# zenghjian/SceneSplat

Hardware: AMD Instinct MI355X
Metric: Gaussians/s encoder fwd+bwd, 102k-pt chunks (higher is better)
Workload: dtype bf16

## Files before the change

include/scenesplat_hip.h:

```cpp
#ifndef SCENESPLAT_HIP_H
#define SCENESPLAT_HIP_H
#include <stddef.h>
#include <stdint.h>

#ifdef __cplusplus
extern "C" {
#endif

struct ihipStream_t;
typedef struct ihipStream_t* ss_stream_t;

#define SS_MAX_ORDERS 8
enum { SS_ORDER_Z = 0, SS_ORDER_Z_TRANS = 1, SS_ORDER_HILBERT = 2, SS_ORDER_HILBERT_TRANS = 3 };
enum { SS_DTYPE_F32 = 0, SS_DTYPE_BF16 = 1 };
enum { SS_ATTN_SIMT = 0, SS_ATTN_MFMA = 1 };
enum { SS_OK = 0, SS_ERR_ARG = 1, SS_ERR_LAUNCH = 2, SS_ERR_WORKSPACE = 3 };

int ss_version(void);

int ss_serialize_encode(const int32_t* grid_coord, const int32_t* batch, int64_t n, int depth, const int* orders,
                        int num_orders, int64_t* codes, ss_stream_t stream);
int ss_offsets_to_batch(const int32_t* offsets, int num_batches, int64_t n, int32_t* batch, ss_stream_t stream);
int ss_count_duplicates(const int64_t* sorted_keys, int64_t n, int32_t* count, ss_stream_t stream);
int ss_grid_coord_max(const int32_t* grid_coord, int64_t n, int32_t* out_max, ss_stream_t stream);
// ... 61 lines not shown
int ss_window_attn_hm_bwd(const void* hm, const void* out, const void* dout, const float* neg_lse2, const int32_t* gidx,
                          const int32_t* sidx, const int32_t* win_start, int num_windows, int max_window, int64_t n,
                          int64_t n_pad, int channels, int num_heads, float scale, void* dqkv, void* workspace,
                          size_t workspace_bytes, ss_stream_t stream);

int ss_window_attn_rpe_fwd(const void* qkv, const int32_t* gidx, const int32_t* sidx, const int32_t* win_start,
                           int num_windows, int max_window, int64_t n, int64_t n_pad, int channels, int num_heads,
                           float scale, int dtype, int impl, const int32_t* grid_coord, const float* table, int pos_bnd,
                           void* out, float* lse, ss_stream_t stream);
size_t ss_window_attn_rpe_bwd_workspace_bytes(int64_t n, int64_t n_pad, int channels, int num_heads, int dtype,
                                              int num_windows, int max_window, int pos_bnd);
int ss_window_attn_rpe_bwd(const void* qkv, const void* out, const void* dout, const float* lse, const int32_t* gidx,
                           const int32_t* sidx, const int32_t* win_start, int num_windows, int max_window, int64_t n,
                           int64_t n_pad, int channels, int num_heads, float scale, int dtype, int impl,
                           const int32_t* grid_coord, const float* table, int pos_bnd, void* dqkv, float* dtable,
                           void* workspace, size_t workspace_bytes, ss_stream_t stream);

int ss_subm_rulebook(const int32_t* grid_coord, const int32_t* batch, int64_t n, int depth,
                     const int64_t* zkeys_sorted, const int32_t* zorder, int swap_xy, int kernel_size, int32_t* nbr,
                     ss_stream_t stream);
int ss_subm_tap_mask_keys(const int32_t* nbr, const int32_t* order, int64_t n, int taps, int coarse_bits, int64_t* keys,
                          ss_stream_t stream);
int64_t ss_subm_rulebook_table_size(int64_t n);
int ss_subm_rulebook_hashed(const int32_t* grid_coord, const int32_t* batch, int64_t n, int depth, int kernel_size, int32_t* nbr,
                            void* workspace, size_t workspace_bytes, ss_stream_t stream);

int ss_subm_conv_fwd(const void* in, const void* weight, const float* bias, const int32_t* nbr, const int32_t* rowperm,
                     void* out, int64_t n, int cin, int cout, int taps, int out_dtype, ss_stream_t stream);
int ss_subm_weight_mirror(const void* w, void* wt, int cout, int taps, int cin, ss_stream_t stream);
int ss_stream_create_cu_mask(int nwords, const uint32_t* mask, void** stream_out);
int ss_subm_im2col(const void* src, const int32_t* nbr, void* dst, int64_t n, int taps, int64_t row_bytes, ss_stream_t stream);
int ss_gemm8_ok(int64_t m, int k, int n, int taps);
int ss_subm_conv_fwd_pipe(const void* in, const void* weight, const float* bias, const int32_t* nbr, const int32_t* rowperm,
                          void* out, int64_t n, int cin, int cout, int taps, int out_dtype, ss_stream_t stream);
int ss_subm_conv_fwd_pipe_walk(const void* in, const void* weight, const float* bias, const int32_t* nbr_walk, const int32_t* rowperm,
                               void* out, int64_t n, int cin, int cout, int taps, int out_dtype, ss_stream_t stream);
int ss_subm_conv_fwd_uses_pipe(int64_t n, int cin, int cout, int taps);
int ss_subm_conv_fwd_walk(const void* in, const void* weight, const float* bias, const int32_t* nbr, const int32_t* nbr_walk,
                          const int32_t* rowperm, void* out, int64_t n, int cin, int cout, int taps, int out_dtype, ss_stream_t stream);
int ss_linear_fwd(const void* x, const void* weight, const float* bias, void* out, int64_t m, int k, int n, int out_dtype,
                  ss_stream_t stream);
int ss_wgrad_xcd_order(void);
int ss_wgrad_set_xcd_order(int on);
int ss_wgrad8_ok(int64_t n, int cin, int cout, int taps);
int ss_subm_conv_wgrad_pipe(const void* in, const void* dout, const int32_t* nbr, const int32_t* rowperm,
                            const int32_t* blk_count, const int32_t* blk_list, float* dweight, int64_t n, int cin, int cout,
                            int taps, ss_stream_t stream);
int ss_linear_wgrad(const void* x, const void* dy, float* dweight, float* dbias, int64_t m, int k_in, int n_out,
                    ss_stream_t stream);
int ss_linear_wgrad_group_plan(int64_t m, int k_in, int n_out, int64_t* desc_words);
int ss_linear_wgrad_tiles(int k_in, int n_out);
int ss_linear_wgrad_group_plan2(int64_t m, int k_in, int n_out, int launch_tiles, int64_t* desc_words);
int ss_linear_wgrad_group(const int64_t* desc, const int32_t* wg_start, int nprob, int total_workgroups, ss_stream_t stream);
int ss_subm_conv_splits(int64_t n, int cout, int taps);
int ss_subm_conv_fwd_splitk(const void* in, const void* weight, const float* bias, const int32_t* nbr, const int32_t* rowperm,
                            float* acc32, int64_t n, int cin, int cout, int taps, int splits, ss_stream_t stream);
int ss_subm_block_lists(const int32_t* nbr, const int32_t* rowperm, int64_t n, int taps, int32_t* blk_count,
                        int32_t* blk_list, ss_stream_t stream);
int ss_subm_conv_wgrad(const void* in, const void* dout, const int32_t* nbr, const int32_t* rowperm,
                       const int32_t* blk_count, const int32_t* blk_list, float* dweight, int64_t n, int cin, int cout,
                       int taps, ss_stream_t stream);

int ss_subm_f32_ok(int cin_padded, int cout);
int ss_subm_f32_fwd(const float* in, const float* wq, const float* bias, const int32_t* nbr_walk, const int32_t* rowperm,
                    float* out, int64_t n, int cin_padded, int cout, int taps, ss_stream_t stream);
int ss_subm_f32_dgrad_dup(const float* dout_folded, const float* wq, const int32_t* nbr_walk, const int32_t* rowperm, float* din,
                          int64_t n, int cin_padded, int cout, int taps, ss_stream_t stream);
int ss_subm_f32_wgrad(const float* in, const float* dout, const int32_t* nbr_walk, const int32_t* rowperm,
                      const int32_t* blk_count, const int32_t* blk_list, float* dweight, int64_t n, int cin_padded,
                      int cin, int cout, int taps, ss_stream_t stream);

int ss_subm_conv_wgrad_pipe_walk(const void* in, const void* dout, const int32_t* nbr_walk, const int32_t* rowperm,
                                 const int32_t* blk_count, const int32_t* blk_list, float* dweight, int64_t n, int cin, int cout,
                                 int taps, ss_stream_t stream);
int ss_subm_conv_wgrad_uses_pipe(int64_t n, int cin, int cout, int taps);
int ss_subm_conv_wgrad_walk(const void* in, const void* dout, const int32_t* nbr, const int32_t* nbr_walk, const int32_t* rowperm,
                            const int32_t* blk_count, const int32_t* blk_list, float* dweight, int64_t n, int cin, int cout,
                            int taps, ss_stream_t stream);

int ss_add_layernorm_fwd(const void* x, int x_dtype, const void* y, int y_dtype, const float* rowscale,
                         const float* gamma, const float* beta, float eps, void* xout, int xout_dtype, void* xcopy_bf16,
                         void* h, int h_dtype, float* mean, float* rstd, int64_t n, int channels, ss_stream_t stream);
int ss_ln_add_ln_fwd(const void* x, int x_dtype, const void* t, int t_dtype, const float* gamma0, const float* beta0, float eps0,
                     const float* gamma1, const float* beta1, float eps1, float* xout, void* h, int h_dtype, float* stats,
                     int64_t n, int channels, ss_stream_t stream);
int ss_ln_add_ln_bwd(const float* g_xout, const void* g_h, int g_h_dtype, const float* xout, const void* t, int t_dtype,
                     const float* stats, const float* gamma0, const float* gamma1, void* g_x, int g_x_dtype, void* g_t,
                     int g_t_dtype, float* part, int64_t n, int channels, int nblocks, ss_stream_t stream);
int ss_add_layernorm_bwd_blocks(int64_t n);

int ss_block_tail_rows(void);
int ss_block_tail_bwd_blocks(int64_t n);
int ss_block_tail_fwd(const void* feat, const float* x, const float* rs1, const float* rs2, const void* wp, const void* bp,
                      const void* w1, const void* b1, const void* w2, const void* b2, int bias_dtype, const float* gamma, const float* beta,
                      float eps, float* x_mid, float* mean, float* rstd, void* h2, void* u, void* a, float* x_out,
                      void* xcopy_bf16, int64_t n, int channels, ss_stream_t stream);
int ss_block_tail_bwd(const float* g_xout, const void* g_xcopy_bf16, const float* x_mid, const float* mean, const float* rstd,
                      const void* u, const float* rs1, const float* rs2, const float* gamma, const void* wp_t, const void* w1_t,
                      const void* w2_t, float* g_mid, void* dfeat, void* dy2, void* du, void* dy1, float* part, int64_t n,
                      int channels, int nblocks, ss_stream_t stream);
int ss_group_partial_sums_outputs_per_workgroup(void);
int ss_group_partial_sums(const int64_t* desc, const int32_t* wg_start, int nprob, int total_workgroups, ss_stream_t stream);
int ss_transpose16_group(const int64_t* desc, const int32_t* wg_start, int nprob, int total_workgroups, ss_stream_t stream);
int ss_subm_weight_mirror_group_tile(void);
int ss_subm_weight_mirror_group(const int64_t* desc, const int32_t* wg_start, int nprob, int total_workgroups, ss_stream_t stream);
int ss_add_layernorm_bwd(const void* g_xout, int g_xout_dtype, const void* g_xcopy, int g_xcopy_dtype, const void* g_h,
// ... 204 lines not shown
```

scenesplat_amd/csrc/wgrad8.hip:

```cpp
#include "grouped.h"
#include <stdlib.h>

typedef __attribute__((ext_vector_type(8))) __bf16 w8_bf8_t;
typedef __attribute__((ext_vector_type(4))) short w8_s4_t;
typedef __attribute__((ext_vector_type(8))) short w8_s8_t;
typedef __attribute__((address_space(3))) w8_s4_t w8_lds_s4_t;
#define W8_MFMA(a, b, c) __builtin_amdgcn_mfma_f32_16x16x32_bf16((a), (b), (c), 0, 0, 0)

#define W8_BUF 65536
#define W8_HALF 16384
#define W8_OFF_B 32768
#define W8_CHUNK 60
#define W8_OFF_ISITE 131072
#define W8_OFF_JSITE (W8_OFF_ISITE + W8_CHUNK * 64 * 4)
#define W8_LDS_BYTES (W8_OFF_JSITE + W8_CHUNK * 64 * 4)
#define W8_ZERO_ELEMS 4096

__device__ uint4 w8_zero[W8_ZERO_ELEMS / 8];

__device__ __forceinline__ void w8_glds16(const void* gsrc, unsigned lds_wave_base) {
  asm volatile("s_mov_b32 m0, %1\n\ts_nop 0\n\tglobal_load_lds_dwordx4 %0, off" ::"v"(gsrc), "s"(lds_wave_base) : "memory");
}
__device__ __forceinline__ w8_bf8_t w8_tr2(const char* p) {
  w8_s4_t lo = __builtin_amdgcn_ds_read_tr16_b64_v4i16((w8_lds_s4_t*)(p));
// ... 239 lines not shown
      }
  if (do_bias && lq == 0) {
#pragma unroll
    for (int ha = 0; ha < 2; ++ha)
#pragma unroll
      for (int r = 0; r < 4; ++r) {
        const int co = m0 + 128 * wr + 64 * ha + 16 * wc + 4 * g + r;
        if (co < Cout) atomicAdd(dbias + co, accb[ha][r]);
      }
  }
}

#undef W8_BIAS

#define W8_XG 3
__device__ __forceinline__ int w8_xcd_order(int L, int nb) {
  const int row = 8 * W8_XG, full = nb / row * row;
  if (L >= full) return L;
  const int xcd = L & 7, slot = L >> 3;
  return ((slot / W8_XG) * 8 + xcd) * W8_XG + slot % W8_XG;
}

template <bool GATHER>
__global__ void __launch_bounds__(512)
k_wgrad8(const unsigned short* __restrict__ X, const unsigned short* __restrict__ DY, const int32_t* __restrict__ nbr,
         const int32_t* __restrict__ rowperm, const int32_t* __restrict__ blk_count, const int32_t* __restrict__ blk_list,
         float* __restrict__ dW, float* __restrict__ dbias, int n, int Cin, int Cout, int taps, int ntn, int nblocks_total,
         int min_per, int ntiles, int nshares, int walk) {
  int L = (int)blockIdx.x;
  if (walk & 2) L = w8_xcd_order(L, (int)gridDim.x);
  w8_body<GATHER>(X, DY, nbr, rowperm, blk_count, blk_list, dW, dbias, n, Cin, Cout, taps, ntn, nblocks_total, min_per, ntiles,
                  nshares, L, walk & 1);
}

__global__ void __launch_bounds__(512)
k_wgrad8_group(const int64_t* __restrict__ desc, const int32_t* __restrict__ wg_start, int nprob, int nprob_flags) {
  const int b = blockIdx.x;
  const int p = group_owner(wg_start, nprob, b);
  const int64_t* d = desc + (int64_t)p * 8;
  const int64_t m = d[4];
  const uint64_t w5 = (uint64_t)d[5], w6 = (uint64_t)d[6], w7 = (uint64_t)d[7];
  const int k_in = (int)(w5 & 0xffffffffu), n_out = (int)(w5 >> 32);
  const int ntn = (int)(w6 & 0xffffffffu), ntiles = (int)(w6 >> 32);
  const int nshares = (int)(w7 & 0xffffffffu), min_per = (int)(w7 >> 32);
  int L = b - wg_start[p];
  if (nprob_flags & 1) {
    const int a = (8 - (wg_start[p] & 7)) & 7;
    if (L >= a) L = a + w8_xcd_order(L - a, nshares * ntiles - a);
  }
  w8_body<false>((const unsigned short*)d[0], (const unsigned short*)d[1], nullptr, nullptr, nullptr, nullptr, (float*)d[2],
                 (float*)d[3], (int)m, k_in, n_out, 1, ntn, (int)((m + 63) / 64), min_per, ntiles, nshares, L);
}

static int w8_xcd_flag = -1;
extern "C" int ss_wgrad_xcd_order(void) {
  if (w8_xcd_flag < 0) { const char* e = getenv("SS_WGRAD_XCD_TRIPLE"); w8_xcd_flag = (e && atoi(e) == 1) ? 1 : 0; }
  return w8_xcd_flag;
}
extern "C" int ss_wgrad_set_xcd_order(int on) { w8_xcd_flag = on ? 1 : 0; return SS_OK; }

extern "C" int ss_wgrad8_ok(int64_t n, int cin, int cout, int taps) {
  return n > 0 && n < (1LL << 31) && cin >= 8 && (cin & 7) == 0 && cin <= W8_ZERO_ELEMS && cout >= 8 && (cout & 7) == 0 &&
         cout <= W8_ZERO_ELEMS && taps >= 1;
}

static int w8_min_per(int64_t busy_tiles, int64_t est_blocks) {
  int64_t per = busy_tiles * est_blocks / 200;
  if (per < 8) per = 8;
  if (per > 160) per = 160;
  return (int)per;
}

static int w8_conv_launch(const void* in, const void* dout, const int32_t* nbr, const int32_t* rowperm, const int32_t* blk_count,
                          const int32_t* blk_list, float* dweight, int64_t n, int cin, int cout, int taps, int walk, hipStream_t stream);

extern "C" int ss_subm_conv_wgrad_pipe(const void* in, const void* dout, const int32_t* nbr, const int32_t* rowperm,
                                       const int32_t* blk_count, const int32_t* blk_list, float* dweight, int64_t n,
                                       int cin, int cout, int taps, hipStream_t stream) {
  return w8_conv_launch(in, dout, nbr, rowperm, blk_count, blk_list, dweight, n, cin, cout, taps, 0, stream);
}
extern "C" int ss_subm_conv_wgrad_pipe_walk(const void* in, const void* dout, const int32_t* nbr_walk, const int32_t* rowperm,
                                            const int32_t* blk_count, const int32_t* blk_list, float* dweight, int64_t n,
                                            int cin, int cout, int taps, hipStream_t stream) {
  return w8_conv_launch(in, dout, nbr_walk, rowperm, blk_count, blk_list, dweight, n, cin, cout, taps, 1, stream);
}

static int w8_conv_launch(const void* in, const void* dout, const int32_t* nbr, const int32_t* rowperm, const int32_t* blk_count,
                          const int32_t* blk_list, float* dweight, int64_t n, int cin, int cout, int taps, int walk, hipStream_t stream) {
  if (n == 0) return SS_OK;
  if (!ss_wgrad8_ok(n, cin, cout, taps) || !blk_count || !blk_list || !nbr) return SS_ERR_ARG;
  const int nblocks = ss_div_up(n, 64);
  const int tm = ss_div_up(cout, 256), tn = ss_div_up(cin, 256);
  static int env_per = -2;
  if (env_per == -2) { const char* e = getenv("SS_WGRAD_MINPER"); env_per = e ? atoi(e) : -1; }
  int min_per = env_per > 0 ? env_per : w8_min_per((int64_t)tm * tn * ((taps + 2) / 3), (int64_t)nblocks * 7 / 10);
  int splits = ss_div_up(nblocks, min_per);
  if (ss_wgrad_xcd_order()) walk |= 2;
  dim3 g((unsigned)((int64_t)taps * splits * tm * tn));
  SS_LAUNCH((k_wgrad8<true>), g, dim3(512), 0, stream, (const unsigned short*)in, (const unsigned short*)dout, nbr, rowperm,
            blk_count, blk_list, dweight, (float*)nullptr, (int)n, cin, cout, taps, tn, nblocks, min_per, tm * tn, splits, walk);
  return SS_OK;
}

static void w8_linear_plan(int64_t m, int k_in, int n_out, int* tm_, int* tn_, int* min_per_, int* splits_, int launch_tiles = 0) {
  const int nblocks = ss_div_up(m, 64);
  const int tm = ss_div_up(n_out, 256), tn = ss_div_up(k_in, 256);
  static int env_per = -2;
  if (env_per == -2) { const char* e = getenv("SS_WGRAD_MINPER"); env_per = e ? atoi(e) : -1; }
  static const int cus = [] {
    int dev = 0, n = 256;
    if (hipGetDevice(&dev) == hipSuccess) (void)hipDeviceGetAttribute(&n, hipDeviceAttributeMultiprocessorCount, dev);
    return n > 0 ? n : 256;
  }();
  const int tiles_all = launch_tiles > tm * tn ? launch_tiles : tm * tn;
  const int shares = cus / tiles_all > 0 ? cus / tiles_all : 1;
  int min_per = env_per > 0 ? env_per : (int)((nblocks + shares - 1) / shares);
  if (env_per <= 0 && min_per < 8) min_per = 8;
  if (min_per > nblocks) min_per = nblocks;
  *tm_ = tm; *tn_ = tn; *min_per_ = min_per; *splits_ = ss_div_up(nblocks, min_per);
}

extern "C" int ss_linear_wgrad_tiles(int k_in, int n_out) { return ss_div_up(n_out, 256) * ss_div_up(k_in, 256); }
extern "C" int ss_linear_wgrad_group_plan2(int64_t m, int k_in, int n_out, int launch_tiles, int64_t* desc_words) {
  if (m <= 0 || !ss_wgrad8_ok(m, k_in, n_out, 1) || !desc_words) return 0;
  int tm, tn, min_per, splits;
  w8_linear_plan(m, k_in, n_out, &tm, &tn, &min_per, &splits, launch_tiles);
  desc_words[5] = (int64_t)((uint64_t)(uint32_t)k_in | ((uint64_t)(uint32_t)n_out << 32));
  desc_words[6] = (int64_t)((uint64_t)(uint32_t)tn | ((uint64_t)(uint32_t)(tm * tn) << 32));
  desc_words[7] = (int64_t)((uint64_t)(uint32_t)splits | ((uint64_t)(uint32_t)min_per << 32));
  return splits * tm * tn;
}
extern "C" int ss_linear_wgrad_group_plan(int64_t m, int k_in, int n_out, int64_t* desc_words) {
  return ss_linear_wgrad_group_plan2(m, k_in, n_out, 0, desc_words);
}

extern "C" int ss_linear_wgrad_group(const int64_t* desc, const int32_t* wg_start, int nprob, int total_workgroups,
                                     hipStream_t stream) {
  SS_GROUP_GUARD(desc, wg_start, nprob, total_workgroups);
  if (nprob > 128) return SS_ERR_ARG;
  SS_LAUNCH(k_wgrad8_group, dim3((unsigned)total_workgroups), dim3(512), 0, stream, desc, wg_start, nprob, 0);
  return SS_OK;
}

extern "C" int ss_linear_wgrad(const void* x, const void* dy, float* dweight, float* dbias, int64_t m, int k_in, int n_out,
                               hipStream_t stream) {
  if (m == 0) return SS_OK;
  if (!ss_wgrad8_ok(m, k_in, n_out, 1)) return SS_ERR_ARG;
  const int nblocks = ss_div_up(m, 64);
  int tm, tn, min_per, splits;
  w8_linear_plan(m, k_in, n_out, &tm, &tn, &min_per, &splits);
  dim3 g((unsigned)(splits * tm * tn));
  SS_LAUNCH((k_wgrad8<false>), g, dim3(512), 0, stream, (const unsigned short*)x, (const unsigned short*)dy,
            (const int32_t*)nullptr, (const int32_t*)nullptr, (const int32_t*)nullptr, (const int32_t*)nullptr, dweight,
            dbias, (int)m, k_in, n_out, 1, tn, nblocks, min_per, tm * tn, splits, 0);
  return SS_OK;
}
```

scenesplat_amd/functional.py:

```python
import os
import weakref

import torch
from torch.utils.weak import WeakIdKeyDictionary

from . import native as nv


def _bf16_autocast(x=None):
    return (x is None or x.is_cuda) and torch.is_autocast_enabled() and torch.get_autocast_dtype("cuda") == torch.bfloat16


class _WindowAttention(torch.autograd.Function):
    @staticmethod
    def forward(ctx, qkv, win, num_heads, scale, impl):
        qkv = qkv.contiguous()
        out, lse = nv.window_attn_fwd(qkv, win, num_heads, scale, impl)
        ctx.save_for_backward(qkv, out, lse)
        ctx.win, ctx.num_heads, ctx.scale, ctx.impl = win, num_heads, scale, impl
        return out

    @staticmethod
    def backward(ctx, dout):
        qkv, out, lse = ctx.saved_tensors
# ... 495 lines not shown
        nv.subm_weight_mirror_group(pairs)


def register_mirrored(weights):
    for p in weights:
        ent = _SHADOW.get(p)
        if ent is not None and p.dim() == 5 and p.shape[-1] % 8 == 0:
            cout, cin = p.shape[0], p.shape[-1]
            ent.want("m", (cin, p.numel() // (cout * cin), cout), p.device)


def register_transposed(weights):
    for p in weights:
        ent = _SHADOW.get(p)
        if ent is not None and p.dim() == 2:
            ent.want("t", (p.shape[1], p.shape[0]), p.device)


def unregister_transposed(weights):
    for ent in filter(None, map(_SHADOW.get, weights)):
        ent.set("t", None)


def unregister_mirrored(weights):
    for ent in filter(None, map(_SHADOW.get, weights)):
        ent.set("m", None)


def mirrored_of(p):
    ent = _current(p)
    return ent.m if ent is not None else None


def bf16_t_of(p):
    ent = _current(p)
    return ent.t if ent is not None else None


def bf16_of(p):
    if p is None or p.dtype == torch.bfloat16:
        return p
    ent = _current(p)
    return ent.bf16 if ent is not None else p.to(torch.bfloat16)


WGRAD_GROUP_MAX_ROWS = int(os.environ.get("SS_WGRAD_GROUP_MAX", str(1 << 22)))
_STAGE = {"cur": None, "route": {}}
_UNFLUSHED = set()


WGRAD_GROUP_MAX_BYTES = int(float(os.environ.get("SS_WGRAD_GROUP_MAX_GIB", "8")) * (1 << 30))


class _WgradStage:
    def __init__(self):
        self.queue = []
        self.redq = []
        self.bytes = 0

    def add(self, x, dy, dw, db):
        self.queue.append((x, dy, dw, db))
        self.bytes += x.numel() * x.element_size() + dy.numel() * dy.element_size()
        if self.bytes > WGRAD_GROUP_MAX_BYTES:
            q, self.queue, self.bytes = self.queue, [], 0
            nv.linear_wgrad_group(q)

    def flush(self):
        _UNFLUSHED.discard(self)
        q, self.queue, self.bytes = self.queue, [], 0
        r, self.redq = self.redq, []
        nv.linear_wgrad_group(q)
        nv.group_partial_sums(r)


class _StageParams(torch.autograd.Function):
    @staticmethod
    def forward(ctx, stage, *params):
        ctx.stage = stage
        ctx.set_materialize_grads(False)
        return tuple(p.view_as(p) for p in params)

    @staticmethod
    def backward(ctx, *grads):
        ctx.stage.flush()
        return (None,) + grads


def stage_begin(linears, n_rows):
    _STAGE["cur"], _STAGE["route"] = None, {}
    if not (WGRAD_GROUP_MAX_ROWS and LINEAR_WGRAD_MIN_ROWS <= n_rows <= WGRAD_GROUP_MAX_ROWS and torch.is_grad_enabled() and _bf16_autocast()):
        return
    params = [p for m in linears for p in (m.weight, m.bias) if p is not None and p.requires_grad and p.dtype == torch.float32 and p.is_cuda]
    if not params:
        return
    stage = _WgradStage()
    aliases = _StageParams.apply(stage, *params)
    _STAGE["cur"], _STAGE["route"] = stage, {id(p): a for p, a in zip(params, aliases)}


def stage_end():
    _STAGE["cur"], _STAGE["route"] = None, {}


def reset_state():
    stage_end()
    _UNFLUSHED.clear()
    _HEAD_CACHE.clear()


def _routed(p):
    a = _STAGE["route"].get(id(p)) if (p is not None and _STAGE["route"]) else None
    return (a, _STAGE["cur"]) if a is not None else (p, None)


def _linear_operands(weight, bias, cast_bias=True):
    wr, stage = _routed(weight) if torch.is_grad_enabled() else (weight, None)
    br = _routed(bias)[0] if stage is not None else bias
    return wr, br, bf16_of(weight), bf16_of(bias) if cast_bias else None, stage, bf16_t_of(weight)


class _Linear(torch.autograd.Function):

    @staticmethod
    def forward(ctx, x, weight, bias, w16, b16, stage, w16t=None):
        y = torch.nn.functional.linear(x, w16, b16)
        _save_linear(ctx, x, weight, bias, w16, w16t, stage)
        return y

    @staticmethod
    def backward(ctx, dy):
        x, w16 = ctx.saved_tensors
        return _linear_backward_of(ctx, x, w16, dy.contiguous()) + (None,) * 4


class _LinearGelu(torch.autograd.Function):

    @staticmethod
    def forward(ctx, x, weight, bias, w16, b16, stage, w16t=None):
        u = torch.nn.functional.linear(x, w16, b16)
        _save_linear(ctx, x, weight, bias, w16, w16t, stage, u)
        return nv.gelu(u)

    @staticmethod
    def backward(ctx, dy):
        x, w16, u = ctx.saved_tensors
        dy = dy.contiguous()
        if not _aligned16(dy):
            dy = dy.clone()
        return _linear_backward_of(ctx, x, w16, nv.gelu(u, dy)) + (None,) * 4


def _save_linear(ctx, x, weight, bias, w16, w16t, stage, *more):
    ctx.save_for_backward(x, w16 if w16t is None else w16t, *more)
    ctx.meta, ctx.dgrad_nt, ctx.stage = (weight.dtype, bias is not None), w16t is not None, stage


def _linear_backward_of(ctx, x, w16, dy):
    w_dtype, has_bias = ctx.meta
    return _linear_backward(x, w16, ctx.dgrad_nt, w_dtype, has_bias, ctx.stage, dy, *ctx.needs_input_grad[:3])

# ... 475 lines not shown
```

scenesplat_amd/native.py:

```python
import ctypes

import numpy as np
import torch

from . import _lib, grouped
from ._lib import check

_C = _lib.CONSTANTS
F32, BF16 = _C["SS_DTYPE_F32"], _C["SS_DTYPE_BF16"]
ATTN_SIMT, ATTN_MFMA = _C["SS_ATTN_SIMT"], _C["SS_ATTN_MFMA"]
HAVE_MFMA_ATTN = True
ORDER_IDS = {name: _C["SS_ORDER_" + name.upper().replace("-", "_")] for name in ("z", "z-trans", "hilbert", "hilbert-trans")}


def _p(t):
    return ctypes.c_void_p(t.data_ptr()) if t is not None else ctypes.c_void_p(0)


def _stream():
    return ctypes.c_void_p(torch.cuda.current_stream().cuda_stream)


def _req(t, dtype=None, name="tensor", shape=None):
    if not isinstance(t, torch.Tensor) or not t.is_cuda:
# ... 305 lines not shown
def dup_fold_rows(src, runs):
    keys, order = runs
    n, C = src.shape
    _req(src, None, "src"); _req(keys, torch.int64, "sorted_keys", (n,)); _req(order, torch.int32, "order", (n,))
    out = torch.empty_like(src)
    check(lib().ss_dup_fold_rows(_p(src), _p(keys), _p(order), _p(out), n, C, dtype_code(src), _stream()), "ss_dup_fold_rows")
    return out


def dup_zero_rows_(x, runs):
    keys, order = runs
    n = x.shape[0]
    _req(x, None, "x"); _req(keys, torch.int64, "sorted_keys", (n,)); _req(order, torch.int32, "order", (n,))
    check(lib().ss_dup_zero_rows(_p(keys), _p(order), _p(x), n, x.shape[1] * x.element_size(), _stream()), "ss_dup_zero_rows")
    return x


def subm_f32_wgrad(x, dout, nbr, rowperm, blocks, cin):
    n, cp = x.shape
    taps = nbr.shape[0]
    _req(x, torch.float32, "x"); _req(dout, torch.float32, "dout", (n, 32)); _req(nbr, torch.int32, "nbr", (taps, n))
    if rowperm is not None:
        _req(rowperm, torch.int32, "rowperm", (n,))
    cnt, lst = blocks
    _req(cnt, torch.int32, "blk_count", (taps,)); _req(lst, torch.int32, "blk_list", (taps, (n + 63) // 64))
    dw = zeros_f32(32 * taps * cin, x.device).view(32, taps, cin)
    check(lib().ss_subm_f32_wgrad(_p(x), _p(dout), _p(nbr), _p(rowperm), _p(cnt), _p(lst), _p(dw), n, cp, cin, 32, taps, _stream()),
          "ss_subm_f32_wgrad")
    return dw


def subm_conv_wgrad_pipe(x, dout, nbr, rowperm, blocks):
    n, cin = x.shape
    cout, taps = dout.shape[1], nbr.shape[0]
    dw = torch.zeros((cout, taps, cin), dtype=torch.float32, device=x.device)
    cnt, lst = blocks
    check(lib().ss_subm_conv_wgrad_pipe(_p(x), _p(dout), _p(nbr), _p(rowperm), _p(cnt), _p(lst), _p(dw), n, cin, cout, taps,
                                        _stream()), "ss_subm_conv_wgrad_pipe")
    return dw


def linear_wgrad_alloc(k, nout, want_bias, device):
    buf = zeros_f32(nout * k + (nout if want_bias else 0), device)
    return buf[:nout * k].view(nout, k), (buf[nout * k:] if want_bias else None)


def linear_wgrad_into(x, dy, dw, db):
    m, k = x.shape
    nout = dy.shape[1]
    _req(x, torch.bfloat16, "x"); _req(dy, torch.bfloat16, "dy", (m, nout)); _req(dw, torch.float32, "dw", (nout, k))
    check(lib().ss_linear_wgrad(_p(x), _p(dy), _p(dw), _p(db), m, k, nout, _stream()), "ss_linear_wgrad")


def linear_wgrad_group(items):
    if not items:
        return
    dev = items[0][0].device
    desc = np.zeros((len(items), 8), dtype=np.int64)
    counts = []
    launch_tiles = sum(lib().ss_linear_wgrad_tiles(x.shape[1], dy.shape[1]) for x, dy, _, _ in items)
    for x, dy, dw, db in items:
        _req(x, torch.bfloat16, "x"); _req(dy, torch.bfloat16, "dy", (x.shape[0], dy.shape[1]))
        _req(dw, torch.float32, "dw", (dy.shape[1], x.shape[1]))
        if db is not None:
            _req(db, torch.float32, "db", (dy.shape[1],))
        j = len(counts)
        nwg = lib().ss_linear_wgrad_group_plan2(x.shape[0], x.shape[1], dy.shape[1], launch_tiles, ctypes.c_void_p(desc[j].ctypes.data))
        if nwg <= 0 or j >= 128:
            linear_wgrad_into(x, dy, dw, db)
            continue
        desc[j, 0], desc[j, 1], desc[j, 2] = x.data_ptr(), dy.data_ptr(), dw.data_ptr()
        desc[j, 3] = db.data_ptr() if db is not None else 0
        desc[j, 4] = x.shape[0]
        counts.append(nwg)
    if counts:
        grouped.launch("ss_linear_wgrad_group", desc[:len(counts)].copy(), grouped.starts(counts), dev)


def linear_wgrad(x, dy, want_bias=False):
    m, k = x.shape
    nout = dy.shape[1]
    _req(x, torch.bfloat16, "x"); _req(dy, torch.bfloat16, "dy", (m, nout))
    buf = zeros_f32(nout * k + (nout if want_bias else 0), x.device)
    dw = buf[:nout * k].view(nout, k)
    db = buf[nout * k:] if want_bias else None
    check(lib().ss_linear_wgrad(_p(x), _p(dy), _p(dw), _p(db), m, k, nout, _stream()), "ss_linear_wgrad")
    return (dw, db) if want_bias else dw


def _dt(t):
    return dtype_code(t) if t is not None else 0


def add_layernorm_fwd(x, y, rowscale, gamma, beta, eps, want_xout, want_copy, h_dtype):
    n, C = x.shape
    _req(x, None, "x")
    if y is not None:
        _req(y, None, "y", (n, C))
    if rowscale is not None:
        _req(rowscale, torch.float32, "rowscale", (n,))
    dev = x.device
    xout = torch.empty((n, C), dtype=torch.float32, device=dev) if want_xout else None
    xcopy = torch.empty((n, C), dtype=torch.bfloat16, device=dev) if want_copy else None
    h = mean = rstd = None
    if gamma is not None:
        _req(gamma, torch.float32, "gamma", (C,)); _req(beta, torch.float32, "beta", (C,))
        h = torch.empty((n, C), dtype=h_dtype, device=dev)
        mean = torch.empty(n, dtype=torch.float32, device=dev); rstd = torch.empty(n, dtype=torch.float32, device=dev)
    check(lib().ss_add_layernorm_fwd(_p(x), _dt(x), _p(y), _dt(y), _p(rowscale), _p(gamma), _p(beta), float(eps), _p(xout), F32,
                                     _p(xcopy), _p(h), _dt(h), _p(mean), _p(rstd), n, C, _stream()), "ss_add_layernorm_fwd")
    return xout, xcopy, h, mean, rstd


def ln_add_ln_fwd(x, t, gamma0, beta0, eps0, gamma1, beta1, eps1, h_dtype):
    n, C = x.shape
    _req(x, None, "x"); _req(t, None, "t", (n, C))
    for p_, nm in ((gamma0, "gamma0"), (beta0, "beta0"), (gamma1, "gamma1"), (beta1, "beta1")):
        _req(p_, torch.float32, nm, (C,))
    dev = x.device
    xout = torch.empty((n, C), dtype=torch.float32, device=dev)
    h = torch.empty((n, C), dtype=h_dtype, device=dev)
    stats = torch.empty((n, 4), dtype=torch.float32, device=dev)
    check(lib().ss_ln_add_ln_fwd(_p(x), _dt(x), _p(t), _dt(t), _p(gamma0), _p(beta0), float(eps0), _p(gamma1), _p(beta1), float(eps1),
                                 _p(xout), _p(h), _dt(h), _p(stats), n, C, _stream()), "ss_ln_add_ln_fwd")
    return xout, h, stats


def group_partial_sums(items):
    if not items:
# ... 1334 lines not shown
```

scenesplat_amd/pointcept_api/ptv3.py:

```python
import os
from functools import partial
from types import SimpleNamespace

import torch
import torch.nn as nn
import torch.nn.functional as F

from .. import functional as SF
from .. import native as nv
from ..plan import build_plan
from .pdnorm import PDNorm, PointModule, ResolvedNorm, pdnorm_layers, resolved as _rn
from .registry import MODELS
from .structure import Point

RUNTIME = dict(attn_impl=nv.ATTN_SIMT, conv_dtype=None,
               attn_headmajor=os.environ.get("SS_ATTN_HM", "1") != "0",
               param_shadows=os.environ.get("SS_PARAM_SHADOWS", "1") != "0",
               fuse_block_tail=os.environ.get("SS_BLOCK_TAIL", "1") != "0")


def bench_runtime():
    return dict(attn_impl=nv.ATTN_MFMA, conv_dtype=torch.bfloat16,
                conv_split_max_channels=int(os.environ.get("SS_CONV_SPLIT_MAX", "32")))

# ... 498 lines not shown
            blocks += [(getattr(enc, f"block{i}"), levels[s].n) for i in range(self.enc_depths[s])]
        if not self.cls_mode and with_dec:
            for s in reversed(range(self.num_stages - 1)):
                dec = getattr(self.dec, f"dec{s}")
                blocks += [(getattr(dec, f"block{i}"), levels[s].n) for i in range(self.dec_depths[s])]
        segs = []
        for blk, n in blocks:
            dp = blk.drop_path[0]
            if isinstance(dp, DropPath) and dp.p > 0.0:
                segs += [(blk, n, 1.0 - dp.p)] * 2
            blk.__dict__["_row_scales"] = []
        if not segs:
            return
        key = tuple((n, k) for _, n, k in segs) + (str(device),)
        cache = self.__dict__.get("_keep_vec")
        if cache is None or cache[0] != key:
            kv = torch.cat([torch.full((n,), k, dtype=torch.float32) for _, n, k in segs]).pin_memory().to(device, non_blocking=True)
            cache = (key, kv)
            self.__dict__["_keep_vec"] = cache
        kv = cache[1]
        scales = nv.row_keep_scales(kv)
        off = 0
        for blk, n, _ in segs:
            blk.__dict__["_row_scales"].append(scales[off:off + n])
            off += n

    def _begin_forward(self, data_dict, perms=None, with_dec=True):
        point = data_dict if isinstance(data_dict, Point) else Point(data_dict)
        feat = point["feat"]
        if not feat.is_cuda:
            raise RuntimeError("PT-v3m1 (scenesplat_amd) runs on the GPU only: the HIP path has no CPU fallback")
        if "grid_coord" not in point:
            if not {"grid_size", "coord"} <= set(point.keys()):
                raise KeyError("need grid_coord, or coord + grid_size (structure.py:54-62)")
            c = point["coord"]
            point["grid_coord"] = torch.div(c - c.min(0)[0], point["grid_size"], rounding_mode="trunc").int()
        if dict.__contains__(point, "offset"):
            offset = point["offset"]
        else:
            offset = point["offset"]
        self._want_copy = (RUNTIME["conv_dtype"] == torch.bfloat16)
        if (torch.is_autocast_enabled() or self._want_copy) and RUNTIME.get("param_shadows", True):
            self._refresh_shadows()
        plan = point.get("plan", None)
        if plan is None:
            plan = build_plan(point["grid_coord"], offset, self.order, self.stride,
                              perms if perms is not None else self.draw_perms())
        elif plan.ready_event is not None:
            torch.cuda.current_stream().wait_event(plan.ready_event)
            plan.record_stream(torch.cuda.current_stream())
            plan.ready_event = None
        if self.training:
            self._draw_row_scales(plan.levels, feat.device, *(() if with_dec else (False,)))
        return point, feat, plan

    def forward(self, data_dict, perms=None):
        point, feat, plan = self._begin_forward(data_dict, perms)
        if self._pdnorm():
            self._resolve_pdnorm(point)
            try:
                return self._forward_levels(point, feat, plan)
            finally:
                for m in self._pdnorm():
                    m.__dict__.pop("_resolved", None)
        return self._forward_levels(point, feat, plan)

    def _forward_levels(self, point, feat, plan):
        x, skips = self._forward_encoder(feat, plan)
        lv = self.num_stages - 1
        if not self.cls_mode:
            x = self._forward_decoder(point, x, skips, plan)
            lv = 0
        out = Point(feat=x, plan=plan, level=lv)
        for k in ("coord", "grid_coord", "offset"):
            if lv == 0 and dict.__contains__(point, k):
                out[k] = point[k]
        return out

    def _embedded(self, x, plan):
        return x

    def _forward_encoder(self, feat, plan):
        levels = plan.levels
        x = self._embedded(self.embedding(feat, levels[0]), plan)
        skips = []
        for s in range(self.num_stages):
            enc = getattr(self.enc, f"enc{s}")
            SF.stage_begin(self._stage_linears(enc), levels[s].n)
            if s > 0:
                skips.append(x)
                x = enc.down(x, levels[s])
            xb = None
            for i in range(self.enc_depths[s]):
                wc = self._want_copy and conv_dtype_for(x.shape[1]) == torch.bfloat16
                x, xb = getattr(enc, f"block{i}")(x, x if xb is None else xb, levels[s], wc and i + 1 < self.enc_depths[s])
            SF.stage_end()
        return x, skips

    def _forward_decoder(self, point, x, skips, plan):
        levels = plan.levels
        cut = point.get("backward_cut", None) if torch.is_grad_enabled() else None
        for s in reversed(range(self.num_stages - 1)):
            dec = getattr(self.dec, f"dec{s}")
            if cut is not None and s == 0 and x.requires_grad:
                leaves = (x.detach().requires_grad_(True), skips[0].detach().requires_grad_(True))
                cut.extend([(x, leaves[0]), (skips[0], leaves[1])])
# ... 11 lines not shown
```

Measured before the change: 2.876 million.

## Overlap deferred large-stage linear weight gradients on a side stream with capped workgroups

Weight-gradient GEMMs for large-row stages are deferred and launched on a side stream using a new persistent-style capped kernel that occupies only part of the CUs. This lets them run concurrently with the backward of subsequent small stages, which would otherwise underfill the GPU. The work is joined back to the main stream later or in an autograd callback. It adds stream synchronisation, bookkeeping, and a host-side tile-split search, and it risks contention or incorrect gradient aliasing when hooks are present.

Measured after the change: 2.945 million, median of 6. 2.4% higher.

```diff
diff --git a/include/scenesplat_hip.h b/include/scenesplat_hip.h
--- a/include/scenesplat_hip.h
+++ b/include/scenesplat_hip.h
@@ -137,6 +137,9 @@
 int ss_linear_wgrad_tiles(int k_in, int n_out);
 int ss_linear_wgrad_group_plan2(int64_t m, int k_in, int n_out, int launch_tiles, int64_t* desc_words);
 int ss_linear_wgrad_group(const int64_t* desc, const int32_t* wg_start, int nprob, int total_workgroups, ss_stream_t stream);
+int ss_linear_wgrad_group_plan_capped(int64_t m, int k_in, int n_out, int launch_tiles, int max_workgroups, int64_t* desc_words);
+int ss_linear_wgrad_group_capped(const int64_t* desc, const int32_t* wg_start, int nprob, int total_items, int max_workgroups,
+                                 ss_stream_t stream);
 int ss_subm_conv_splits(int64_t n, int cout, int taps);
 int ss_subm_conv_fwd_splitk(const void* in, const void* weight, const float* bias, const int32_t* nbr, const int32_t* rowperm,
                             float* acc32, int64_t n, int cin, int cout, int taps, int splits, ss_stream_t stream);
diff --git a/scenesplat_amd/csrc/wgrad8.hip b/scenesplat_amd/csrc/wgrad8.hip
--- a/scenesplat_amd/csrc/wgrad8.hip
+++ b/scenesplat_amd/csrc/wgrad8.hip
@@ -315,6 +315,22 @@
                  (float*)d[3], (int)m, k_in, n_out, 1, ntn, (int)((m + 63) / 64), min_per, ntiles, nshares, L);
 }
 
+__global__ void __launch_bounds__(512)
+k_wgrad8_group_capped(const int64_t* __restrict__ desc, const int32_t* __restrict__ wg_start, int nprob, int total_items) {
+  for (int b = blockIdx.x; b < total_items; b += (int)gridDim.x) {
+    const int p = group_owner(wg_start, nprob, b);
+    const int64_t* d = desc + (int64_t)p * 8;
+    const int64_t m = d[4];
+    const uint64_t w5 = (uint64_t)d[5], w6 = (uint64_t)d[6], w7 = (uint64_t)d[7];
+    const int k_in = (int)(w5 & 0xffffffffu), n_out = (int)(w5 >> 32);
+    const int ntn = (int)(w6 & 0xffffffffu), ntiles = (int)(w6 >> 32);
+    const int nshares = (int)(w7 & 0xffffffffu), min_per = (int)(w7 >> 32);
+    w8_body<false>((const unsigned short*)d[0], (const unsigned short*)d[1], nullptr, nullptr, nullptr, nullptr, (float*)d[2],
+                   (float*)d[3], (int)m, k_in, n_out, 1, ntn, (int)((m + 63) / 64), min_per, ntiles, nshares, b - wg_start[p]);
+    __syncthreads();
+  }
+}
+
 static int w8_xcd_flag = -1;
 extern "C" int ss_wgrad_xcd_order(void) {
   if (w8_xcd_flag < 0) { const char* e = getenv("SS_WGRAD_XCD_TRIPLE"); w8_xcd_flag = (e && atoi(e) == 1) ? 1 : 0; }
@@ -397,6 +413,36 @@
   return ss_linear_wgrad_group_plan2(m, k_in, n_out, 0, desc_words);
 }
 
+#define W8_CAP_ROUNDS 4
+extern "C" int ss_linear_wgrad_group_plan_capped(int64_t m, int k_in, int n_out, int launch_tiles, int max_workgroups,
+                                                 int64_t* desc_words) {
+  if (m <= 0 || max_workgroups <= 0 || !ss_wgrad8_ok(m, k_in, n_out, 1) || !desc_words) return 0;
+  const int nblocks = ss_div_up(m, 64);
+  const int tm = ss_div_up(n_out, 256), tn = ss_div_up(k_in, 256);
+  const int64_t tiles_all = launch_tiles > tm * tn ? launch_tiles : tm * tn;
+  int64_t shares = (int64_t)W8_CAP_ROUNDS * max_workgroups / tiles_all;
+  if (shares < 1) shares = 1;
+  if (shares > nblocks / 8) shares = nblocks / 8 > 0 ? nblocks / 8 : 1;
+  int min_per = nblocks, splits = 1;
+  for (int s = (int)shares; s > 1; --s) {
+    const int per = ss_div_up(nblocks, s), n = ss_div_up(nblocks, per);
+    if (nblocks - (n - 1) * per >= 8) { min_per = per; splits = n; break; }
+  }
+  desc_words[5] = (int64_t)((uint64_t)(uint32_t)k_in | ((uint64_t)(uint32_t)n_out << 32));
+  desc_words[6] = (int64_t)((uint64_t)(uint32_t)tn | ((uint64_t)(uint32_t)(tm * tn) << 32));
+  desc_words[7] = (int64_t)((uint64_t)(uint32_t)splits | ((uint64_t)(uint32_t)min_per << 32));
+  return splits * tm * tn;
+}
+
+extern "C" int ss_linear_wgrad_group_capped(const int64_t* desc, const int32_t* wg_start, int nprob, int total_items,
+                                            int max_workgroups, hipStream_t stream) {
+  SS_GROUP_GUARD(desc, wg_start, nprob, total_items);
+  if (nprob > 128 || max_workgroups <= 0) return SS_ERR_ARG;
+  const int grid = total_items < max_workgroups ? total_items : max_workgroups;
+  SS_LAUNCH(k_wgrad8_group_capped, dim3((unsigned)grid), dim3(512), 0, stream, desc, wg_start, nprob, total_items);
+  return SS_OK;
+}
+
 extern "C" int ss_linear_wgrad_group(const int64_t* desc, const int32_t* wg_start, int nprob, int total_workgroups,
                                      hipStream_t stream) {
   SS_GROUP_GUARD(desc, wg_start, nprob, total_workgroups);
diff --git a/scenesplat_amd/functional.py b/scenesplat_amd/functional.py
--- a/scenesplat_amd/functional.py
+++ b/scenesplat_amd/functional.py
@@ -571,11 +571,95 @@
 WGRAD_GROUP_MAX_BYTES = int(float(os.environ.get("SS_WGRAD_GROUP_MAX_GIB", "8")) * (1 << 30))
 
 
+WGRAD_OVERLAP = os.environ.get("SS_WGRAD_OVERLAP", "1") != "0"
+WGRAD_DEFER_MIN_ROWS = int(os.environ.get("SS_WGRAD_DEFER_MIN_ROWS", "16384"))
+WGRAD_OVERLAP_FREE_CUS = int(os.environ.get("SS_WGRAD_OVERLAP_FREE_CUS", "80"))
+_OVERLAP = {"armed": False, "stages": [], "items": [], "pairs": [], "held": [], "flight": None, "callback": False, "streams": {}}
+OVERLAP_STATS = {"deferred": 0, "launched": 0, "joined": 0}
+
+
+def wgrad_overlap_arm(on):
+    if _OVERLAP["flight"] is not None or _OVERLAP["items"] or _OVERLAP["held"]:
+        _overlap_clear()
+    _OVERLAP["armed"] = bool(on) and WGRAD_OVERLAP and WGRAD_DEFER_MIN_ROWS > 0
+    _OVERLAP["stages"] = []
+
+
+def _overlap_clear():
+    flight = _OVERLAP["flight"]
+    if flight is not None and not torch.cuda.is_current_stream_capturing():
+        flight[0].wait_stream(flight[1])
+    _OVERLAP.update(armed=False, stages=[], items=[], pairs=[], held=[], flight=None, callback=False)
+
+
+def _overlap_alias(stage, q):
+    q = [(x, dy, dw.detach(), db.detach() if db is not None else None) for x, dy, dw, db in q]
+    stage.late = stage.late or {}
+    stage.late.update({t.data_ptr(): t for _, _, dw, db in q for t in (dw, db) if t is not None})
+    if not _OVERLAP["callback"]:
+        _OVERLAP["callback"] = True
+        torch.autograd.Variable._execution_engine.queue_callback(_overlap_finish)
+    return q
+
+
+def _overlap_launch():
+    items, _OVERLAP["items"] = _OVERLAP["items"], []
+    main = torch.cuda.current_stream()
+    dev = items[0][0].device
+    side = _OVERLAP["streams"].get(dev)
+    if side is None:
+        side = _OVERLAP["streams"][dev] = torch.cuda.Stream(dev)
+    side.wait_stream(main)
+    cus = torch.cuda.get_device_properties(dev).multi_processor_count
+    nv.linear_wgrad_group(items, max_workgroups=max(1, cus - WGRAD_OVERLAP_FREE_CUS), stream=side)
+    _OVERLAP["flight"] = (main, side, items)
+    OVERLAP_STATS["launched"] += 1
+
+
+def _overlap_join():
+    flight, _OVERLAP["flight"] = _OVERLAP["flight"], None
+    held, _OVERLAP["held"] = _OVERLAP["held"], []
+    if flight is None:
+        return None
+    main = flight[0]
+    with torch.cuda.stream(main):
+        main.wait_stream(flight[1])
+        for stage, q in held:
+            nv.linear_wgrad_group(q)
+            stage.late = None
+    OVERLAP_STATS["joined"] += 1
+    return main
+
+
+def _overlap_finish():
+    try:
+        cur = torch.cuda.current_stream()
+        if _OVERLAP["items"]:
+            items, _OVERLAP["items"] = _OVERLAP["items"], []
+            nv.linear_wgrad_group(items)
+        main = _overlap_join() or cur
+        if cur != main:
+            cur.wait_stream(main)
+        for p, g in _OVERLAP["pairs"]:
+            if p.grad is None or p.grad.data_ptr() != g.data_ptr():
+                raise RuntimeError("a deferred weight gradient was copied before it was computed (a gradient hook?): "
+                                   "run with SS_WGRAD_OVERLAP=0")
+    finally:
+        _overlap_clear()
+
+
 class _WgradStage:
-    def __init__(self):
+    def __init__(self, n_rows=0, params=()):
         self.queue = []
         self.redq = []
         self.bytes = 0
+        self.n_rows = n_rows
+        self.params = params
+        self.defer = False
+        self.prev = None
+        self.late = None
+        self.flushed = False
+        self.hooked = True
 
     def add(self, x, dy, dw, db):
         self.queue.append((x, dy, dw, db))
@@ -588,7 +672,21 @@
         _UNFLUSHED.discard(self)
         q, self.queue, self.bytes = self.queue, [], 0
         r, self.redq = self.redq, []
-        nv.linear_wgrad_group(q)
+        first, self.flushed = not self.flushed, True
+        flight = _OVERLAP["flight"] is not None
+        late_ok = (q and (self.defer or flight) and not self.hooked and not torch.is_grad_enabled()
+                   and all(p.grad is None for p in self.params))
+        if late_ok and self.defer and not flight:
+            _OVERLAP["items"] += _overlap_alias(self, q)
+            OVERLAP_STATS["deferred"] += 1
+            if self.prev is None or not self.prev.defer:
+                _overlap_launch()
+        elif late_ok:
+            _OVERLAP["held"].append((self, _overlap_alias(self, q)))
+        else:
+            nv.linear_wgrad_group(q)
+        if flight and first and (self.prev is None or max(self.n_rows, self.prev.n_rows) >= WGRAD_DEFER_MIN_ROWS):
+            _overlap_join()
         nv.group_partial_sums(r)
 
 
@@ -601,18 +699,36 @@
 
     @staticmethod
     def backward(ctx, *grads):
-        ctx.stage.flush()
+        stage = ctx.stage
+        stage.flush()
+        ptrs, stage.late = stage.late, None
+        if ptrs:
+            _OVERLAP["pairs"] += [(p, ptrs[g.data_ptr()]) for p, g in zip(stage.params, grads) if g is not None and g.data_ptr() in ptrs]
         return (None,) + grads
+
+
+def _overlap_enter(stage, hooked):
+    stages = _OVERLAP["stages"]
+    stage.defer = (bool(stage.params) and stage.n_rows >= WGRAD_DEFER_MIN_ROWS and not hooked
+                   and any(st.n_rows < WGRAD_DEFER_MIN_ROWS for st in stages))
+    stage.hooked = hooked
+    stage.prev = stages[-1] if stages else None
+    stages.append(stage)
 
 
 def stage_begin(linears, n_rows):
     _STAGE["cur"], _STAGE["route"] = None, {}
-    if not (WGRAD_GROUP_MAX_ROWS and LINEAR_WGRAD_MIN_ROWS <= n_rows <= WGRAD_GROUP_MAX_ROWS and torch.is_grad_enabled() and _bf16_autocast()):
+    params = []
+    if WGRAD_GROUP_MAX_ROWS and LINEAR_WGRAD_MIN_ROWS <= n_rows <= WGRAD_GROUP_MAX_ROWS and torch.is_grad_enabled() and _bf16_autocast():
+        params = [p for m in linears for p in (m.weight, m.bias) if p is not None and p.requires_grad and p.dtype == torch.float32 and p.is_cuda]
+    if not params:
+        if _OVERLAP["armed"]:
+            _overlap_enter(_WgradStage(n_rows), False)
         return
-    params = [p for m in linears for p in (m.weight, m.bias) if p is not None and p.requires_grad and p.dtype == torch.float32 and p.is_cuda]
-    if not params:
-        return
-    stage = _WgradStage()
+    stage = _WgradStage(n_rows, params)
+    if _OVERLAP["armed"]:
+        _overlap_enter(stage, any(getattr(p, "_post_accumulate_grad_hooks", None) or p._backward_hooks for p in params) or (
+            torch.distributed.is_available() and torch.distributed.is_initialized() and torch.distributed.get_world_size() > 1))
     aliases = _StageParams.apply(stage, *params)
     _STAGE["cur"], _STAGE["route"] = stage, {id(p): a for p, a in zip(params, aliases)}
 
@@ -625,6 +741,7 @@
     stage_end()
     _UNFLUSHED.clear()
     _HEAD_CACHE.clear()
+    _overlap_clear()
 
 
 def _routed(p):
diff --git a/scenesplat_amd/native.py b/scenesplat_amd/native.py
--- a/scenesplat_amd/native.py
+++ b/scenesplat_amd/native.py
@@ -381,20 +381,59 @@
     check(lib().ss_linear_wgrad(_p(x), _p(dy), _p(dw), _p(db), m, k, nout, _stream()), "ss_linear_wgrad")
 
 
-def linear_wgrad_group(items):
+_CAPPED_TILES = {}
+
+
+def _capped_launch_tiles(shapes, cap):
+    key = (shapes, cap)
+    if key in _CAPPED_TILES:
+        return _CAPPED_TILES[key]
+    tiles = [lib().ss_linear_wgrad_tiles(k, n) for _, k, n in shapes]
+    kt = [_div_up(m, 64) for m, _, _ in shapes]
+    work = sum(t * b for t, b in zip(tiles, kt))
+    words = np.zeros(8, dtype=np.int64)
+    best = None
+    for rounds in (4, 2, 3, 5, 6, 8):
+        cand = [max(1, _div_up(work * 4, rounds * b)) for b in kt]
+        lengths = []
+        for (m, k, n), lt, t, b in zip(shapes, cand, tiles, kt):
+            if lib().ss_linear_wgrad_group_plan_capped(m, k, n, lt, cap, ctypes.c_void_p(words.ctypes.data)) <= 0:
+                continue
+            shares, per = int(words[7]) & 0xffffffff, int(words[7]) >> 32
+            lengths += [min(per, b - s * per) + 8 for s in range(shares) for _ in range(t)]
+        grid = max(1, min(cap, len(lengths)))
+        span = max(sum(lengths[b::grid]) for b in range(grid)) if lengths else 0
+        if best is None or span < best[0]:
+            best = (span, cand)
+    if len(_CAPPED_TILES) > 64:
+        _CAPPED_TILES.clear()
+    _CAPPED_TILES[key] = best[1]
+    return best[1]
+
+
+def linear_wgrad_group(items, max_workgroups=None, stream=None):
     if not items:
         return
+    if stream is not None:
+        with torch.cuda.stream(stream):
+            return linear_wgrad_group(items, max_workgroups)
     dev = items[0][0].device
     desc = np.zeros((len(items), 8), dtype=np.int64)
     counts = []
     launch_tiles = sum(lib().ss_linear_wgrad_tiles(x.shape[1], dy.shape[1]) for x, dy, _, _ in items)
+    if max_workgroups is not None:
+        capped_tiles = _capped_launch_tiles(tuple((x.shape[0], x.shape[1], dy.shape[1]) for x, dy, _, _ in items[:128]), int(max_workgroups))
     for x, dy, dw, db in items:
         _req(x, torch.bfloat16, "x"); _req(dy, torch.bfloat16, "dy", (x.shape[0], dy.shape[1]))
         _req(dw, torch.float32, "dw", (dy.shape[1], x.shape[1]))
         if db is not None:
             _req(db, torch.float32, "db", (dy.shape[1],))
         j = len(counts)
-        nwg = lib().ss_linear_wgrad_group_plan2(x.shape[0], x.shape[1], dy.shape[1], launch_tiles, ctypes.c_void_p(desc[j].ctypes.data))
+        words = ctypes.c_void_p(desc[j].ctypes.data)
+        if max_workgroups is None:
+            nwg = lib().ss_linear_wgrad_group_plan2(x.shape[0], x.shape[1], dy.shape[1], launch_tiles, words)
+        else:
+            nwg = lib().ss_linear_wgrad_group_plan_capped(x.shape[0], x.shape[1], dy.shape[1], capped_tiles[len(counts)], int(max_workgroups), words)
         if nwg <= 0 or j >= 128:
             linear_wgrad_into(x, dy, dw, db)
             continue
@@ -402,8 +441,10 @@
         desc[j, 3] = db.data_ptr() if db is not None else 0
         desc[j, 4] = x.shape[0]
         counts.append(nwg)
-    if counts:
+    if counts and max_workgroups is None:
         grouped.launch("ss_linear_wgrad_group", desc[:len(counts)].copy(), grouped.starts(counts), dev)
+    elif counts:
+        grouped.launch("ss_linear_wgrad_group_capped", desc[:len(counts)].copy(), grouped.starts(counts), dev, int(max_workgroups))
 
 
 def linear_wgrad(x, dy, want_bias=False):
diff --git a/scenesplat_amd/pointcept_api/ptv3.py b/scenesplat_amd/pointcept_api/ptv3.py
--- a/scenesplat_amd/pointcept_api/ptv3.py
+++ b/scenesplat_amd/pointcept_api/ptv3.py
@@ -574,6 +574,7 @@
             plan.ready_event = None
         if self.training:
             self._draw_row_scales(plan.levels, feat.device, *(() if with_dec else (False,)))
+        SF.wgrad_overlap_arm(self.training and torch.is_grad_enabled() and point.get("backward_cut", None) is None)
         return point, feat, plan
 
     def forward(self, data_dict, perms=None):
```
